# yshen47/SGAM_NeurIPS22

Measured on AMD Instinct MI355X. Metric: generated RGB-D frames/sec (256x256, GoogleEarth), higher is better.
Workload: dtype f32; 1 GPU; GoogleEarth-Infinite 256x256 inference loop (BASELINE configs[2]): forward-splat warp (N<=3) + VQGAN encode/quantise(4096)/decode + frame feedback, in-HBM frame store; frames_per_gpu=1105, scenes=1, parallelism=scene-parallel x1, launch=hip-graph replay of the VQGAN forward, f32_products=exact hi/lo fp16 split on the fp16 matrix cores, fp32 accumulate

## Files before the change

sgam_neurips22_amd/csrc/attention.hip:

```cpp
#include "sgam_common.h"

namespace {

typedef unsigned int u32x4 __attribute__((ext_vector_type(4)));
typedef unsigned int u32x2 __attribute__((ext_vector_type(2)));
typedef _Float16 f16x8 __attribute__((ext_vector_type(8)));

constexpr int AD = 256;
constexpr int KB = 32;
constexpr int BLK_BYTES = KB * AD * 4;
constexpr float P_LIFT = 10.0f;
constexpr float LOG2E = 1.4426950408889634f;
constexpr float RESCALE_TAU = 5.0f;

__device__ __forceinline__ f32x16 mfma16(u32x4 a, u32x4 b, f32x16 c) {
    return __builtin_amdgcn_mfma_f32_32x32x16_f16(__builtin_bit_cast(f16x8, a), __builtin_bit_cast(f16x8, b), c, 0, 0, 0);
}

__device__ __forceinline__ void split8(const float *v, u32x4 &hi, u32x4 &lo) {
#pragma unroll
    for (int e = 0; e < 4; ++e) {
        const _Float16 h0 = (_Float16)v[2 * e], h1 = (_Float16)v[2 * e + 1];
        const _Float16 l0 = (_Float16)(v[2 * e] - (float)h0), l1 = (_Float16)(v[2 * e + 1] - (float)h1);
        hi[e] = (unsigned)__builtin_bit_cast(unsigned short, h0) | ((unsigned)__builtin_bit_cast(unsigned short, h1) << 16);
        lo[e] = (unsigned)__builtin_bit_cast(unsigned short, l0) | ((unsigned)__builtin_bit_cast(unsigned short, l1) << 16);
    }
}

__global__ __launch_bounds__(256) void attn_split_kv_kernel(const float *__restrict__ k, const float *__restrict__ v, int ld,
                                                            int n, unsigned short *__restrict__ kf,
                                                            unsigned short *__restrict__ vf) {
    const int gid = blockIdx.x * 256 + threadIdx.x;
    const int row = gid & 31, h = (gid >> 5) & 1, t = (gid >> 6) & 1, tile = (gid >> 7) & 7, kb = gid >> 10;
    if (kb * KB >= n) return;
    float kv[8], vv[8];
    const float *kp = k + (int64_t)(kb * KB + row) * ld + tile * 32 + t * 16 + h * 8;
    const f32x4 k0 = *reinterpret_cast<const f32x4 *>(kp), k1 = *reinterpret_cast<const f32x4 *>(kp + 4);
#pragma unroll
    for (int e = 0; e < 4; ++e) {
        kv[e] = k0[e];
        kv[4 + e] = k1[e];
    }
#pragma unroll
    for (int s = 0; s < 8; ++s) {
        const int key = 4 * h + 8 * (2 * t + (s >> 2)) + (s & 3);
        vv[s] = v[(int64_t)(kb * KB + key) * ld + tile * 32 + row];
    }
    u32x4 hi, lo;
    const int64_t piece = ((int64_t)(kb * 8 + tile) * 256 + (t * 2 + h) * 32 + row) * 8;
    split8(kv, hi, lo);
    *reinterpret_cast<u32x4 *>(kf + piece) = hi;
    *reinterpret_cast<u32x4 *>(kf + piece + 128 * 8) = lo;
    split8(vv, hi, lo);
    *reinterpret_cast<u32x4 *>(vf + piece) = hi;
    *reinterpret_cast<u32x4 *>(vf + piece + 128 * 8) = lo;
}

struct AttnParams {
    const unsigned short *qf;
    const float *q;
    const unsigned short *kf, *vf;
    float *ws_o;
    float *ws_ml;
    int ld, n, blocks_per_split;
    int n_img, nsplit;
    float qscale;
};

constexpr int NSPLIT = 8;

typedef __attribute__((address_space(1))) const void gptr_t;
typedef __attribute__((address_space(3))) void lptr_t;

__global__ __launch_bounds__(256) void attn_flash_f32x_kernel(const AttnParams p) {
    __shared__ __attribute__((aligned(16))) unsigned char smem[4 * BLK_BYTES];
    const int tid = threadIdx.x, lane = tid & 63, wave = tid >> 6;
    const int sp = blockIdx.x % p.nsplit, qb = blockIdx.x / p.nsplit;
    const int q0 = qb * 128 + wave * 32;
    const int lq = lane & 31, lh = lane >> 5;
    const int kb0 = ((qb * 128) / p.n_img) * (p.n_img / KB) + sp * p.blocks_per_split, kb1 = kb0 + p.blocks_per_split;
    const unsigned char *kg = reinterpret_cast<const unsigned char *>(p.kf), *vg = reinterpret_cast<const unsigned char *>(p.vf);

    const int wave_s = __builtin_amdgcn_readfirstlane(wave);
    auto dma1 = [&](const unsigned char *g, int kb, int slot, const int i) {
        const unsigned char *src = g + (int64_t)kb * BLK_BYTES + wave_s * 8192 + (i >> 2) * 4096 + lane * 16;
        unsigned char *dst = smem + slot * BLK_BYTES + wave_s * 8192 + (i >> 2) * 4096;
        switch (i & 3) {
        case 0: __builtin_amdgcn_global_load_lds((gptr_t *)src, (lptr_t *)dst, 16, 0, 0); break;
        case 1: __builtin_amdgcn_global_load_lds((gptr_t *)src, (lptr_t *)dst, 16, 1024, 0); break;
        case 2: __builtin_amdgcn_global_load_lds((gptr_t *)src, (lptr_t *)dst, 16, 2048, 0); break;
        default: __builtin_amdgcn_global_load_lds((gptr_t *)src, (lptr_t *)dst, 16, 3072, 0); break;
        }
    };
    auto dma = [&](const unsigned char *g, int kb, int slot) {
#pragma unroll
        for (int i = 0; i < 8; ++i) dma1(g, kb, slot, i);
    };
    u32x4 qh[16], ql[16];
    if (p.qf) {
        const unsigned short *qb = p.qf + (int64_t)(q0 >> 5) * (16 * 1024) + lane * 8;
#pragma unroll
        for (int t = 0; t < 16; ++t) {
            qh[t] = *reinterpret_cast<const u32x4 *>(qb + t * 1024);
            ql[t] = *reinterpret_cast<const u32x4 *>(qb + t * 1024 + 512);
        }
    } else {
        const float *qp = p.q + (int64_t)(q0 + lq) * p.ld + lh * 8;
#pragma unroll
        for (int t = 0; t < 16; ++t) {
            const f32x4 a = *reinterpret_cast<const f32x4 *>(qp + t * 16), b = *reinterpret_cast<const f32x4 *>(qp + t * 16 + 4);
            float v[8];
#pragma unroll
            for (int e = 0; e < 4; ++e) {
                v[e] = a[e] * p.qscale;
                v[4 + e] = b[e] * p.qscale;
            }
            split8(v, qh[t], ql[t]);
        }
    }

    f32x16 o[8];
#pragma unroll
    for (int i = 0; i < 8; ++i)
#pragma unroll
        for (int e = 0; e < 16; ++e) o[i][e] = 0.f;
    float m_run = -INFINITY, l_run = 0.f;

    const int nb = kb1 - kb0;
    auto blk = [&](int j) { return kb0 + (j < nb ? j : nb - 1); };
    dma(kg, blk(0), 0);
    dma(vg, blk(0), 2);
    dma(kg, blk(1), 1);

    u32x4 fh[3], fl[3];
    f32x16 sacc[2];
    float s[16], pe[2];
    u32x4 ph[2], pl[2];
    auto lds_off = [](const unsigned char *ptr) {
        return (unsigned)(uintptr_t)(__attribute__((address_space(3))) const unsigned char *)ptr;
    };
#define ATTN_DS_READ(dst, addr, off) asm volatile("ds_read_b128 %0, %1 offset:%2" : "=v"(dst) : "v"(addr), "i"(off))
#define ATTN_DS_WAIT(n, set) asm volatile("s_waitcnt lgkmcnt(" #n ")" : "+v"(fh[set]), "+v"(fl[set]))
#define ATTN_BARRIER(cnt)                                        \
    do {                                                          \
        asm volatile("s_waitcnt vmcnt(" #cnt ")" ::: "memory");   \
        __builtin_amdgcn_s_barrier();                             \
    } while (0)
    auto smfma = [&](const int t) {
        sacc[(3 * t) & 1] = mfma16(fh[t % 3], qh[t], sacc[(3 * t) & 1]);
        sacc[(3 * t + 1) & 1] = mfma16(fh[t % 3], ql[t], sacc[(3 * t + 1) & 1]);
        sacc[(3 * t + 2) & 1] = mfma16(fl[t % 3], qh[t], sacc[(3 * t + 2) & 1]);
    };
#define ATTN_FRAG(set, base, t)                                              \
    do {                                                                      \
        ATTN_DS_READ(fh[set], base, ((t) >> 1) * 4096 + ((t) & 1) * 1024);        \
        ATTN_DS_READ(fl[set], base, ((t) >> 1) * 4096 + (2 + ((t) & 1)) * 1024);  \
    } while (0)
    ATTN_BARRIER(0);

    {
        const unsigned lk = lds_off(smem + lane * 16);
#pragma unroll
        for (int e = 0; e < 16; ++e) sacc[0][e] = sacc[1][e] = 0.f;
        ATTN_FRAG(0, lk, 0);
        ATTN_FRAG(1, lk, 1);
#pragma unroll
        for (int t = 0; t < 16; ++t) {
            if (t + 2 < 16) ATTN_FRAG((t + 2) % 3, lk, t + 2);
            if (t + 2 < 16) ATTN_DS_WAIT(4, t % 3);
            else if (t + 1 < 16) ATTN_DS_WAIT(2, t % 3);
            else ATTN_DS_WAIT(0, t % 3);
            smfma(t);
        }
        float mloc = -INFINITY;
#pragma unroll
        for (int e = 0; e < 16; ++e) {
            s[e] = (sacc[0][e] + sacc[1][e]) * LOG2E;
            mloc = fmaxf(mloc, s[e]);
        }
        m_run = fmaxf(mloc, __shfl_xor(mloc, 32, 64));
        ATTN_BARRIER(0);
        dma(kg, blk(2), 0);
    }

    for (int j = 0; j < nb; ++j) {
        const int buf = j & 1;
        const unsigned lk = lds_off(smem + (buf ^ 1) * BLK_BYTES + lane * 16);
        const unsigned lv = lds_off(smem + (2 + buf) * BLK_BYTES + lane * 16);
        const int kb_k = blk(j + 3), kb_v = blk(j + 1);
#pragma unroll
        for (int e = 0; e < 16; ++e) sacc[0][e] = sacc[1][e] = 0.f;
        ATTN_FRAG(0, lk, 0);
        ATTN_FRAG(1, lk, 1);
#pragma unroll
        for (int t = 0; t < 16; ++t) {
            if (t + 2 < 16) ATTN_FRAG((t + 2) % 3, lk, t + 2);
            if (t < 8) dma1(vg, kb_v, 2 + (buf ^ 1), t);
            if (t + 2 < 16) ATTN_DS_WAIT(4, t % 3);
            else if (t + 1 < 16) ATTN_DS_WAIT(2, t % 3);
            else ATTN_DS_WAIT(0, t % 3);
            smfma(t);
            pe[t & 1] = __builtin_amdgcn_exp2f(s[t] - m_run + P_LIFT);
            l_run += pe[t & 1];
            if (t & 1) {
                typedef _Float16 f16x2 __attribute__((ext_vector_type(2)));
                const f16x2 h = __builtin_bit_cast(f16x2, __builtin_amdgcn_cvt_pkrtz(pe[0], pe[1]));
                const f16x2 l = __builtin_bit_cast(f16x2, __builtin_amdgcn_cvt_pkrtz(pe[0] - (float)h[0], pe[1] - (float)h[1]));
                ph[t >> 3][(t & 7) >> 1] = __builtin_bit_cast(unsigned, h);
                pl[t >> 3][(t & 7) >> 1] = __builtin_bit_cast(unsigned, l);
            }
        }
        ATTN_BARRIER(16);
        float mloc = -INFINITY;
        ATTN_FRAG(16 % 3, lv, 0);
        ATTN_FRAG(17 % 3, lv, 1);
#pragma unroll
        for (int u = 0; u < 16; ++u) {
            if (u + 2 < 16) ATTN_FRAG((16 + u + 2) % 3, lv, u + 2);
            if (u < 8) dma1(kg, kb_k, buf ^ 1, u);
            if (u + 2 < 16) ATTN_DS_WAIT(4, (16 + u) % 3);
            else if (u + 1 < 16) ATTN_DS_WAIT(2, (16 + u) % 3);
            else ATTN_DS_WAIT(0, (16 + u) % 3);
            const int i = u >> 1, t = u & 1, set = (16 + u) % 3;
            o[i] = mfma16(fh[set], ph[t], o[i]);
            o[i] = mfma16(fh[set], pl[t], o[i]);
            o[i] = mfma16(fl[set], ph[t], o[i]);
            if (u >= 4) {
#pragma unroll
                for (int e = (u - 4) * 4 / 3; e < (u - 3) * 4 / 3; ++e) {
                    s[e] = (sacc[0][e] + sacc[1][e]) * LOG2E;
                    mloc = fmaxf(mloc, s[e]);
                }
            }
        }
        if (j + 1 < nb) {
            mloc = fmaxf(mloc, __shfl_xor(mloc, 32, 64));
            const float m_new = fmaxf(m_run, mloc);
            if (__any(m_new > m_run + RESCALE_TAU)) {
                const float alpha = __builtin_amdgcn_exp2f(m_run - m_new);
                l_run *= alpha;
#pragma unroll
                for (int i = 0; i < 8; ++i)
#pragma unroll
                    for (int e = 0; e < 16; ++e) {
                        float x = o[i][e], tmp;
                        asm volatile("v_accvgpr_read_b32 %1, %0\n\tv_mul_f32 %1, %1, %2\n\tv_accvgpr_write_b32 %0, %1"
                                     : "+a"(x), "=&v"(tmp)
                                     : "v"(alpha));
                        o[i][e] = x;
                    }
                m_run = m_new;
            }
        }
        ATTN_BARRIER(16);
    }
#undef ATTN_FRAG
#undef ATTN_BARRIER
#undef ATTN_DS_WAIT
#undef ATTN_DS_READ

    l_run += __shfl_xor(l_run, 32, 64);
    if (lh == 0) {
        float *ml = p.ws_ml + ((int64_t)sp * p.n + q0 + lq) * 2;
        ml[0] = m_run;
        ml[1] = l_run;
    }
    float *wo = p.ws_o + ((int64_t)sp * (p.n / 32) + (q0 >> 5)) * (AD * 32) + lq;
#pragma unroll
    for (int i = 0; i < 8; ++i)
#pragma unroll
        for (int e = 0; e < 16; ++e)
            wo[(32 * i + 8 * (e >> 2) + 4 * lh + (e & 3)) * 32] = o[i][e];
    asm volatile("s_waitcnt vmcnt(0)" ::: "memory");
}

template <int NS>
__global__ __launch_bounds__(256) void attn_combine_kernel(const float *__restrict__ ws_o, const float *__restrict__ ws_ml,
                                                           float *__restrict__ out, int ldo, int n, int32_t *range_flag) {
    __shared__ float tile[32][33];
    const int qt = blockIdx.x >> 3, dg = blockIdx.x & 7;
    const int q = threadIdx.x & 31, dsub = threadIdx.x >> 5;
    float w[NS], l[NS], o[NS][4], M = -INFINITY, L = 0.f;
#pragma unroll
    for (int s = 0; s < NS; ++s) {
        const float *ml = ws_ml + ((int64_t)s * n + qt * 32 + q) * 2;
        w[s] = ml[0];
        l[s] = ml[1];
    }
#pragma unroll
    for (int s = 0; s < NS; ++s)
#pragma unroll
        for (int j = 0; j < 4; ++j) o[s][j] = ws_o[(((int64_t)s * (n / 32) + qt) * AD + dg * 32 + dsub * 4 + j) * 32 + q];
#pragma unroll
    for (int s = 0; s < NS; ++s) M = fmaxf(M, w[s]);
#pragma unroll
    for (int s = 0; s < NS; ++s) {
        w[s] = __builtin_amdgcn_exp2f(w[s] - M);
        L += w[s] * l[s];
    }
    const float inv = 1.0f / L;
    float acc[4] = {0.f, 0.f, 0.f, 0.f};
#pragma unroll
    for (int s = 0; s < NS; ++s)
#pragma unroll
        for (int j = 0; j < 4; ++j) acc[j] += w[s] * o[s][j];
#pragma unroll
    for (int j = 0; j < 4; ++j) tile[q][dsub * 4 + j] = acc[j] * inv;
    __syncthreads();
    const int r = threadIdx.x >> 3, c4 = (threadIdx.x & 7) * 4;
    const f32x4 v = {tile[r][c4], tile[r][c4 + 1], tile[r][c4 + 2], tile[r][c4 + 3]};
    *reinterpret_cast<f32x4 *>(out + (int64_t)(qt * 32 + r) * ldo + dg * 32 + c4) = v;
    if (range_flag && sgam_not_finite((v[0] + v[1]) + (v[2] + v[3]))) atomicOr(range_flag, 1);
}

struct CombProjParams {
    const float *ws_o, *ws_ml;
    const unsigned short *w;
    const float *bias, *res;
    float *out;
    double *gn_partial;
    int n_img;
    int32_t *range_flag;
    int n, ns, ldr, ldc;
    float inv_w_scale;
};

template <int NS>
__global__ __launch_bounds__(256) void attn_combine_proj_f32x_kernel(const CombProjParams p) {
    constexpr int LDK = AD + 8;
    __shared__ __attribute__((aligned(16))) unsigned short sA[2][32][LDK];
    const int tid = threadIdx.x, lane = tid & 63, wave = tid >> 6;
    const int qt = blockIdx.x;
    const int lr = lane & 31, lh = lane >> 5;
    constexpr int WD = 4, KS = AD / 16, SLABS = AD / 32;
    const unsigned short *wt0 = p.w + (int64_t)(wave * 2) * SLABS * 2048, *wt1 = wt0 + (int64_t)SLABS * 2048;
    u32x4 wh[WD][2], wl[WD][2];
    auto wfrag = [&](int kstep, u32x4 (&hi)[2], u32x4 (&lo)[2]) {
        const int off = (kstep >> 1) * 2048 + (((kstep & 1) * 2 + lh) * 32 + lr) * 8;
        hi[0] = *reinterpret_cast<const u32x4 *>(wt0 + off);
        lo[0] = *reinterpret_cast<const u32x4 *>(wt0 + off + 1024);
        hi[1] = *reinterpret_cast<const u32x4 *>(wt1 + off);
        lo[1] = *reinterpret_cast<const u32x4 *>(wt1 + off + 1024);
    };
    const int q = tid & 31, dg = tid >> 5;
    float w[NS], l[NS], M = -INFINITY, L = 0.f;
#pragma unroll
    for (int s = 0; s < NS; ++s) {
        w[s] = p.ws_ml[((int64_t)s * p.n + qt * 32 + q) * 2];
        l[s] = p.ws_ml[((int64_t)s * p.n + qt * 32 + q) * 2 + 1];
    }
    const float *ob = p.ws_o + ((int64_t)qt * AD + dg * 32) * 32 + q;
    const int64_t sstride = (int64_t)p.n * AD;
    constexpr int CPS = NS >= 8 ? 16 : 32, NSTEP = 32 / CPS;
    for (int s = 0; s < NS; ++s) M = fmaxf(M, w[s]);
#pragma unroll
    for (int s = 0; s < NS; ++s) {
        w[s] = __builtin_amdgcn_exp2f(w[s] - M);
        L += w[s] * l[s];
    }
    const float inv = 1.0f / L;
    bool bad = false;
#pragma unroll
    for (int step = 0; step < NSTEP; ++step) {
        float cur[CPS][NS];
#pragma unroll
        for (int j = 0; j < CPS; ++j)
#pragma unroll
            for (int s = 0; s < NS; ++s) cur[j][s] = ob[s * sstride + (step * CPS + j) * 32];
        float a[CPS];
#pragma unroll
        for (int j = 0; j < CPS; ++j) a[j] = 0.f;
#pragma unroll
        for (int s = 0; s < NS; ++s)
#pragma unroll
            for (int j = 0; j < CPS; ++j) a[j] += w[s] * cur[j][s];
#pragma unroll
        for (int h4 = 0; h4 < CPS / 4; ++h4) {
            unsigned hi[2], lo[2];
#pragma unroll
            for (int e = 0; e < 2; ++e) {
                const float a0 = a[4 * h4 + 2 * e] * inv, a1 = a[4 * h4 + 2 * e + 1] * inv;
                bad |= sgam_not_finite(a0 + a1);
                const _Float16 h0 = (_Float16)a0, h1 = (_Float16)a1;
                const _Float16 l0 = (_Float16)(a0 - (float)h0), l1 = (_Float16)(a1 - (float)h1);
                hi[e] = (unsigned)__builtin_bit_cast(unsigned short, h0) | ((unsigned)__builtin_bit_cast(unsigned short, h1) << 16);
                lo[e] = (unsigned)__builtin_bit_cast(unsigned short, l0) | ((unsigned)__builtin_bit_cast(unsigned short, l1) << 16);
            }
            const int d = dg * 32 + step * CPS + 4 * h4;
            *reinterpret_cast<u32x2 *>(&sA[0][q][d]) = u32x2{hi[0], hi[1]};
            *reinterpret_cast<u32x2 *>(&sA[1][q][d]) = u32x2{lo[0], lo[1]};
        }
    }
    if (bad && p.range_flag) atomicOr(p.range_flag, 1);
#pragma unroll
    for (int t = 0; t < WD; ++t) wfrag(t, wh[t], wl[t]);
    const int m0 = qt * 32;
    float rres[2][16], rbias[2];
#pragma unroll
    for (int j = 0; j < 2; ++j) {
        const int nn = wave * 64 + j * 32 + lr;
        rbias[j] = p.bias ? p.bias[nn] : 0.f;
#pragma unroll
        for (int e = 0; e < 16; ++e) rres[j][e] = p.res ? p.res[(int64_t)(m0 + 8 * (e >> 2) + 4 * lh + (e & 3)) * p.ldr + nn] : 0.f;
    }
    __syncthreads();
    f32x16 acc[2];
#pragma unroll
    for (int j = 0; j < 2; ++j)
#pragma unroll
        for (int e = 0; e < 16; ++e) acc[j][e] = 0.f;
#pragma unroll
    for (int t = 0; t < KS; ++t) {
        u32x4 bh[2] = {wh[t % WD][0], wh[t % WD][1]}, bl[2] = {wl[t % WD][0], wl[t % WD][1]};
        wfrag(t + WD < KS ? t + WD : KS - 1, wh[t % WD], wl[t % WD]);
        __builtin_amdgcn_sched_barrier(0);
        const u32x4 ah = *reinterpret_cast<const u32x4 *>(&sA[0][lr][t * 16 + lh * 8]);
        const u32x4 al = *reinterpret_cast<const u32x4 *>(&sA[1][lr][t * 16 + lh * 8]);
#pragma unroll
        for (int j = 0; j < 2; ++j) {
            acc[j] = mfma16(ah, bh[j], acc[j]);
            acc[j] = mfma16(ah, bl[j], acc[j]);
            acc[j] = mfma16(al, bh[j], acc[j]);
        }
    }
#pragma unroll
    for (int j = 0; j < 2; ++j) {
        const int nn = wave * 64 + j * 32 + lr;
        const float bias = rbias[j];
        float gs = 0.f, gss = 0.f;
#pragma unroll
        for (int e = 0; e < 16; ++e) {
            const int row = m0 + 8 * (e >> 2) + 4 * lh + (e & 3);
            float v = acc[j][e] * p.inv_w_scale + bias;
            v += rres[j][e];
            p.out[(int64_t)row * p.ldc + nn] = v;
            gs += v;
            gss += v * v;
        }
        if (p.range_flag && sgam_not_finite(gs)) atomicOr(p.range_flag, 1);
        if (p.gn_partial) {
            constexpr int CPO = AD / 32;
            double ds = (double)gs, dss = (double)gss;
#pragma unroll
            for (int o = 1; o < CPO; o <<= 1) {
                ds += __shfl_xor(ds, o, 64);
                dss += __shfl_xor(dss, o, 64);
            }
            ds += __shfl_xor(ds, 32, 64);
            dss += __shfl_xor(dss, 32, 64);
            if (lh == 0 && (lr % CPO) == 0) {
                double *o = p.gn_partial + ((int64_t)qt * 32 + nn / CPO) * 2;
                o[0] = ds;
                o[1] = dss;
            }
        }
    }
}

struct QkvXParams {
    const float *x;
    const float *mean_rstd;
    const float *gamma, *beta;
    const unsigned short *w;
    const float *bias;
    unsigned short *qf;
    unsigned short *kf, *vf;
    int32_t *range_flag;
    int ldx, n_img;
    float inv_w_scale, qscale;
};

__global__ __launch_bounds__(256, 2) void attn_qkv_gn_f32x_kernel(const QkvXParams p) {
    constexpr int LDK = AD + 8;
    constexpr int VLD = 64 + 4;
    __shared__ __attribute__((aligned(16))) unsigned short sA[2][64][LDK];
    const int tid = threadIdx.x, lane = tid & 63, wave = tid >> 6;
    const int m0 = blockIdx.x * 64, by = blockIdx.y;
    const int lr = lane & 31, lh = lane >> 5;
    const int b = m0 / p.n_img;
    constexpr int cpg = AD / 32, WD = 4, KS = AD / 16, NIT = 64 * (AD / 4) / 256;
    const unsigned short *wt = p.w + (int64_t)(by * 4 + wave) * (AD / 32) * 2048;
    auto wfrag = [&](int kstep, u32x4 &hi, u32x4 &lo) {
        const unsigned short *q = wt + (int64_t)(kstep >> 1) * 2048 + (((kstep & 1) * 2 + lh) * 32 + lr) * 8;
        hi = *reinterpret_cast<const u32x4 *>(q);
        lo = *reinterpret_cast<const u32x4 *>(q + 1024);
    };
    u32x4 wh[WD], wl[WD];
#pragma unroll
    for (int t = 0; t < WD; ++t) wfrag(t, wh[t], wl[t]);
    {
        const int prow = tid / (AD / 4), pc4 = (tid % (AD / 4)) * 4;
        f32x4 xr[NIT];
#pragma unroll
        for (int it = 0; it < NIT; ++it) xr[it] = *reinterpret_cast<const f32x4 *>(p.x + (int64_t)(m0 + prow + it * 4) * p.ldx + pc4);
        const int g = pc4 / cpg;
        const float mean = p.mean_rstd[(b * 32 + g) * 2], rstd = p.mean_rstd[(b * 32 + g) * 2 + 1];
        const f32x4 ga = *reinterpret_cast<const f32x4 *>(p.gamma + pc4), be = *reinterpret_cast<const f32x4 *>(p.beta + pc4);
#pragma unroll
        for (int it = 0; it < NIT; ++it) {
            const int row = prow + it * 4;
            f32x4 v = xr[it];
#pragma unroll
            for (int e = 0; e < 4; ++e) v[e] = (v[e] - mean) * rstd * ga[e] + be[e];
            unsigned hi[2], lo[2];
#pragma unroll
            for (int e = 0; e < 2; ++e) {
                const float a0 = v[2 * e], a1 = v[2 * e + 1];
                const _Float16 h0 = (_Float16)a0, h1 = (_Float16)a1;
                const _Float16 l0 = (_Float16)(a0 - (float)h0), l1 = (_Float16)(a1 - (float)h1);
                hi[e] = (unsigned)__builtin_bit_cast(unsigned short, h0) | ((unsigned)__builtin_bit_cast(unsigned short, h1) << 16);
                lo[e] = (unsigned)__builtin_bit_cast(unsigned short, l0) | ((unsigned)__builtin_bit_cast(unsigned short, l1) << 16);
            }
            *reinterpret_cast<unsigned long long *>(&sA[0][row][pc4]) = (unsigned long long)hi[0] | ((unsigned long long)hi[1] << 32);
            *reinterpret_cast<unsigned long long *>(&sA[1][row][pc4]) = (unsigned long long)lo[0] | ((unsigned long long)lo[1] << 32);
        }
    }
    f32x16 acc[2];
#pragma unroll
    for (int j = 0; j < 2; ++j)
#pragma unroll
        for (int e = 0; e < 16; ++e) acc[j][e] = 0.f;
    __syncthreads();
#pragma unroll
    for (int t = 0; t < KS; ++t) {
        const u32x4 ah = wh[t % WD], al = wl[t % WD];
        wfrag(t + WD < KS ? t + WD : KS - 1, wh[t % WD], wl[t % WD]);
        __builtin_amdgcn_sched_barrier(0);
#pragma unroll
        for (int j = 0; j < 2; ++j) {
            const u32x4 xh = *reinterpret_cast<const u32x4 *>(&sA[0][j * 32 + lr][t * 16 + lh * 8]);
            const u32x4 xl = *reinterpret_cast<const u32x4 *>(&sA[1][j * 32 + lr][t * 16 + lh * 8]);
            acc[j] = mfma16(ah, xh, acc[j]);
            acc[j] = mfma16(al, xh, acc[j]);
            acc[j] = mfma16(ah, xl, acc[j]);
        }
    }
    const int cw = wave * 32 + 16 * lh;
    float bias[16];
#pragma unroll
    for (int e4 = 0; e4 < 4; ++e4) {
        const f32x4 bv = *reinterpret_cast<const f32x4 *>(p.bias + by * 128 + cw + e4 * 4);
        bias[4 * e4] = bv[0], bias[4 * e4 + 1] = bv[1], bias[4 * e4 + 2] = bv[2], bias[4 * e4 + 3] = bv[3];
    }
    float v[2][16], gs = 0.f;
#pragma unroll
    for (int j = 0; j < 2; ++j)
#pragma unroll
        for (int e = 0; e < 16; ++e) {
            v[j][e] = acc[j][e] * p.inv_w_scale + bias[e];
            gs += v[j][e];
        }
    if (p.range_flag && sgam_not_finite(gs)) atomicOr(p.range_flag, 1);
    if (by < 2) {
#pragma unroll
        for (int j = 0; j < 2; ++j) {
            unsigned short *dst = p.qf + ((int64_t)((m0 >> 5) + j) * 16 + by * 8 + wave * 2 + lh) * 1024 + lr * 8;
#pragma unroll
            for (int h = 0; h < 2; ++h) {
                float sv[8];
#pragma unroll
                for (int e = 0; e < 8; ++e) sv[e] = v[j][8 * h + e] * p.qscale;
                u32x4 hi, lo;
                split8(sv, hi, lo);
                *reinterpret_cast<u32x4 *>(dst + h * 32 * 8) = hi;
                *reinterpret_cast<u32x4 *>(dst + h * 32 * 8 + 512) = lo;
            }
        }
    } else if (by < 4) {
#pragma unroll
        for (int j = 0; j < 2; ++j) {
            const int64_t kb = (m0 >> 5) + j;
            unsigned short *dst = p.kf + ((kb * 8 + (by - 2) * 4 + wave) * 256 + (lh * 2) * 32 + lr) * 8;
#pragma unroll
            for (int h = 0; h < 2; ++h) {
                u32x4 hi, lo;
                split8(&v[j][8 * h], hi, lo);
// ... 1255 lines not shown
```

Baseline: 384.6 frames/s.

## Overlap Q panel loads with first K/V DMA and peel pipeline tail trips

Issues the first K block DMA before loading the Q panel and uses inline-asm global loads with explicit vmcnt waits, so Q loads and K/V prefetch overlap. The main attention loop is split into templated trips that peel the last three iterations, which removes the redundant clamped re-fetches of the final block and the extra S computation after the last block. The final vmcnt(0) is also dropped. This adds finely hand-tuned vmcnt counts, and any miscount could cause a race on LDS or registers.

```diff
diff --git a/sgam_neurips22_amd/csrc/attention.hip b/sgam_neurips22_amd/csrc/attention.hip
--- a/sgam_neurips22_amd/csrc/attention.hip
+++ b/sgam_neurips22_amd/csrc/attention.hip
@@ -1,4 +1,6 @@
 #include "sgam_common.h"
+
+#include <type_traits>
 
 namespace {
 
@@ -96,19 +98,45 @@
 #pragma unroll
         for (int i = 0; i < 8; ++i) dma1(g, kb, slot, i);
     };
+    const int nb = kb1 - kb0;
+    dma(kg, kb0, 0);
     u32x4 qh[16], ql[16];
+#define ATTN_PANEL_LOAD(dst, ptr, off) asm volatile("global_load_dwordx4 %0, %1, off offset:%2" : "=v"(dst) : "v"(ptr), "i"(off) : "memory")
+#define ATTN_PANEL_WAIT(cnt)                                                                                                        \
+    do {                                                                                                                             \
+        asm volatile("s_waitcnt vmcnt(%14)"                                                                                          \
+                     : "+v"(qh[0]), "+v"(qh[1]), "+v"(qh[2]), "+v"(qh[3]), "+v"(qh[4]), "+v"(qh[5]), "+v"(qh[6]), "+v"(qh[7]),       \
+                       "+v"(qh[8]), "+v"(qh[9]), "+v"(qh[10]), "+v"(qh[11]), "+v"(qh[12]), "+v"(qh[13])                              \
+                     : "i"(cnt));                                                                                                    \
+        asm volatile("" : "+v"(qh[14]), "+v"(qh[15]), "+v"(ql[0]), "+v"(ql[1]), "+v"(ql[2]), "+v"(ql[3]), "+v"(ql[4]), "+v"(ql[5]),  \
+                          "+v"(ql[6]), "+v"(ql[7]), "+v"(ql[8]), "+v"(ql[9]), "+v"(ql[10]), "+v"(ql[11]));                           \
+        asm volatile("" : "+v"(ql[12]), "+v"(ql[13]), "+v"(ql[14]), "+v"(ql[15]));                                                   \
+    } while (0)
     if (p.qf) {
         const unsigned short *qb = p.qf + (int64_t)(q0 >> 5) * (16 * 1024) + lane * 8;
 #pragma unroll
         for (int t = 0; t < 16; ++t) {
-            qh[t] = *reinterpret_cast<const u32x4 *>(qb + t * 1024);
-            ql[t] = *reinterpret_cast<const u32x4 *>(qb + t * 1024 + 512);
+            ATTN_PANEL_LOAD(qh[t], qb + t * 1024, 0);
+            ATTN_PANEL_LOAD(ql[t], qb + t * 1024, 1024);
         }
     } else {
         const float *qp = p.q + (int64_t)(q0 + lq) * p.ld + lh * 8;
 #pragma unroll
         for (int t = 0; t < 16; ++t) {
-            const f32x4 a = *reinterpret_cast<const f32x4 *>(qp + t * 16), b = *reinterpret_cast<const f32x4 *>(qp + t * 16 + 4);
+            ATTN_PANEL_LOAD(qh[t], qp + t * 16, 0);
+            ATTN_PANEL_LOAD(ql[t], qp + t * 16, 16);
+        }
+    }
+    if (nb > 1) dma(kg, kb0 + 1, 1);
+    dma(vg, kb0, 2);
+    if (nb == 1) asm volatile("s_waitcnt vmcnt(8)" ::: "memory");
+    ATTN_PANEL_WAIT(16);
+#undef ATTN_PANEL_WAIT
+#undef ATTN_PANEL_LOAD
+    if (!p.qf) {
+#pragma unroll
+        for (int t = 0; t < 16; ++t) {
+            const f32x4 a = __builtin_bit_cast(f32x4, qh[t]), b = __builtin_bit_cast(f32x4, ql[t]);
             float v[8];
 #pragma unroll
             for (int e = 0; e < 4; ++e) {
@@ -126,11 +154,6 @@
         for (int e = 0; e < 16; ++e) o[i][e] = 0.f;
     float m_run = -INFINITY, l_run = 0.f;
 
-    const int nb = kb1 - kb0;
-    auto blk = [&](int j) { return kb0 + (j < nb ? j : nb - 1); };
-    dma(kg, blk(0), 0);
-    dma(vg, blk(0), 2);
-    dma(kg, blk(1), 1);
 
     u32x4 fh[3], fl[3];
     f32x16 sacc[2];
@@ -141,10 +164,10 @@
     };
 #define ATTN_DS_READ(dst, addr, off) asm volatile("ds_read_b128 %0, %1 offset:%2" : "=v"(dst) : "v"(addr), "i"(off))
 #define ATTN_DS_WAIT(n, set) asm volatile("s_waitcnt lgkmcnt(" #n ")" : "+v"(fh[set]), "+v"(fl[set]))
-#define ATTN_BARRIER(cnt)                                        \
-    do {                                                          \
-        asm volatile("s_waitcnt vmcnt(" #cnt ")" ::: "memory");   \
-        __builtin_amdgcn_s_barrier();                             \
+#define ATTN_BARRIER(cnt)                                              \
+    do {                                                                \
+        asm volatile("s_waitcnt vmcnt(%0)" ::"i"(cnt) : "memory");      \
+        __builtin_amdgcn_s_barrier();                                   \
     } while (0)
     auto smfma = [&](const int t) {
         sacc[(3 * t) & 1] = mfma16(fh[t % 3], qh[t], sacc[(3 * t) & 1]);
@@ -156,7 +179,7 @@
         ATTN_DS_READ(fh[set], base, ((t) >> 1) * 4096 + ((t) & 1) * 1024);        \
         ATTN_DS_READ(fl[set], base, ((t) >> 1) * 4096 + (2 + ((t) & 1)) * 1024);  \
     } while (0)
-    ATTN_BARRIER(0);
+    __builtin_amdgcn_s_barrier();
 
     {
         const unsigned lk = lds_off(smem + lane * 16);
@@ -179,27 +202,35 @@
             mloc = fmaxf(mloc, s[e]);
         }
         m_run = fmaxf(mloc, __shfl_xor(mloc, 32, 64));
-        ATTN_BARRIER(0);
-        dma(kg, blk(2), 0);
-    }
-
-    for (int j = 0; j < nb; ++j) {
+        if (nb > 1) {
+            ATTN_BARRIER(8);
+            if (nb > 2) dma(kg, kb0 + 2, 0);
+        }
+    }
+
+    auto trip = [&](const int j, auto tail_c) {
+        constexpr int TAIL = decltype(tail_c)::value;
+        constexpr bool NEXT = TAIL >= 1, REQ_K = TAIL >= 3;
         const int buf = j & 1;
         const unsigned lk = lds_off(smem + (buf ^ 1) * BLK_BYTES + lane * 16);
         const unsigned lv = lds_off(smem + (2 + buf) * BLK_BYTES + lane * 16);
-        const int kb_k = blk(j + 3), kb_v = blk(j + 1);
-#pragma unroll
-        for (int e = 0; e < 16; ++e) sacc[0][e] = sacc[1][e] = 0.f;
-        ATTN_FRAG(0, lk, 0);
-        ATTN_FRAG(1, lk, 1);
+        const int kb_k = kb0 + j + 3, kb_v = kb0 + j + 1;
+        if constexpr (NEXT) {
+#pragma unroll
+            for (int e = 0; e < 16; ++e) sacc[0][e] = sacc[1][e] = 0.f;
+            ATTN_FRAG(0, lk, 0);
+            ATTN_FRAG(1, lk, 1);
+        }
 #pragma unroll
         for (int t = 0; t < 16; ++t) {
-            if (t + 2 < 16) ATTN_FRAG((t + 2) % 3, lk, t + 2);
-            if (t < 8) dma1(vg, kb_v, 2 + (buf ^ 1), t);
-            if (t + 2 < 16) ATTN_DS_WAIT(4, t % 3);
-            else if (t + 1 < 16) ATTN_DS_WAIT(2, t % 3);
-            else ATTN_DS_WAIT(0, t % 3);
-            smfma(t);
+            if constexpr (NEXT) {
+                if (t + 2 < 16) ATTN_FRAG((t + 2) % 3, lk, t + 2);
+                if (t + 2 < 16) ATTN_DS_WAIT(4, t % 3);
+                else if (t + 1 < 16) ATTN_DS_WAIT(2, t % 3);
+                else ATTN_DS_WAIT(0, t % 3);
+                smfma(t);
+                if (t < 8) dma1(vg, kb_v, 2 + (buf ^ 1), t);
+            }
             pe[t & 1] = __builtin_amdgcn_exp2f(s[t] - m_run + P_LIFT);
             l_run += pe[t & 1];
             if (t & 1) {
@@ -210,14 +241,13 @@
                 pl[t >> 3][(t & 7) >> 1] = __builtin_bit_cast(unsigned, l);
             }
         }
-        ATTN_BARRIER(16);
+        ATTN_BARRIER(TAIL >= 2 ? 16 : 8 * TAIL);
         float mloc = -INFINITY;
         ATTN_FRAG(16 % 3, lv, 0);
         ATTN_FRAG(17 % 3, lv, 1);
 #pragma unroll
         for (int u = 0; u < 16; ++u) {
             if (u + 2 < 16) ATTN_FRAG((16 + u + 2) % 3, lv, u + 2);
-            if (u < 8) dma1(kg, kb_k, buf ^ 1, u);
             if (u + 2 < 16) ATTN_DS_WAIT(4, (16 + u) % 3);
             else if (u + 1 < 16) ATTN_DS_WAIT(2, (16 + u) % 3);
             else ATTN_DS_WAIT(0, (16 + u) % 3);
@@ -225,7 +255,8 @@
             o[i] = mfma16(fh[set], ph[t], o[i]);
             o[i] = mfma16(fh[set], pl[t], o[i]);
             o[i] = mfma16(fl[set], ph[t], o[i]);
-            if (u >= 4) {
+            if (REQ_K && u < 8) dma1(kg, kb_k, buf ^ 1, u);
+            if (NEXT && u >= 4) {
 #pragma unroll
                 for (int e = (u - 4) * 4 / 3; e < (u - 3) * 4 / 3; ++e) {
                     s[e] = (sacc[0][e] + sacc[1][e]) * LOG2E;
@@ -233,7 +264,7 @@
                 }
             }
         }
-        if (j + 1 < nb) {
+        if constexpr (NEXT) {
             mloc = fmaxf(mloc, __shfl_xor(mloc, 32, 64));
             const float m_new = fmaxf(m_run, mloc);
             if (__any(m_new > m_run + RESCALE_TAU)) {
@@ -252,8 +283,12 @@
                 m_run = m_new;
             }
         }
-        ATTN_BARRIER(16);
-    }
+        if constexpr (TAIL >= 2) ATTN_BARRIER(TAIL >= 3 ? 16 : 8);
+    };
+    for (int j = 0; j + 3 < nb; ++j) trip(j, std::integral_constant<int, 3>());
+    if (nb >= 3) trip(nb - 3, std::integral_constant<int, 2>());
+    if (nb >= 2) trip(nb - 2, std::integral_constant<int, 1>());
+    trip(nb - 1, std::integral_constant<int, 0>());
 #undef ATTN_FRAG
 #undef ATTN_BARRIER
 #undef ATTN_DS_WAIT
@@ -271,7 +306,6 @@
 #pragma unroll
         for (int e = 0; e < 16; ++e)
             wo[(32 * i + 8 * (e >> 2) + 4 * lh + (e & 3)) * 32] = o[i][e];
-    asm volatile("s_waitcnt vmcnt(0)" ::: "memory");
 }
 
 template <int NS>
```

Result: no change. 385.1 frames/s, median of 6 (+0.1%).
